# sebrahimi1988/dss-ml-at-scale

Measured on NVIDIA H100. Metric: series fitted+forecast/sec, higher is better.
Workload: dtype f32

## Files before the change

dss-ml-at-scale_b200/csrc/fit_tc.cu:

```cuda
#include "mmf_internal.cuh"
#include "sm90_ptx.cuh"

namespace mmf {
namespace {

using namespace sm90;

constexpr int TILE_M = 128;
constexpr int KC = 32;
constexpr int NGROUPS = 2;
constexpr int FOLD_CHUNKS = 18;
constexpr int MAX_PRED = 64;
constexpr int BULK_MAX_PRED = 28;
constexpr int Y_STAGE_BYTES = TILE_M * KC * 4;
constexpr int AT_STAGE_BYTES = 2 * P * KC * 4;
constexpr int THREADS = 416;
constexpr int WARP_EPI0 = 8, WARP_PROD = 12;

template <int STAGES, int OBUF, bool SE = false>
struct SmemLayoutT {
  static constexpr int y = 0;
  static constexpr int at = y + STAGES * Y_STAGE_BYTES;
  static constexpr int apred = at + STAGES * AT_STAGE_BYTES;
  static constexpr int ostage = apred + MAX_PRED * P * 4;
  static constexpr int acc = ostage + OBUF * TILE_M * BULK_MAX_PRED * 4;
  static constexpr int nm = acc + 2 * NGROUPS * TILE_M * P * 4;
  static constexpr int cc = nm + 2 * NGROUPS * TILE_M * 2;
  static constexpr int bars = cc + NGROUPS * 2 * TILE_M * 4;
  static constexpr int n_bars = 2 * STAGES + 4;
  static constexpr int ss = bars + n_bars * 8;
  static constexpr int sfac = ss + (SE ? 2 * NGROUPS * TILE_M * 8 : 0);
  static constexpr int total = sfac + (SE ? MAX_PRED * 4 : 0);
  static_assert(total + 1024 <= 232448, "exceeds the 227 KB of shared memory a CTA can opt into");
};

__device__ __forceinline__ float dot16(const float* __restrict__ arow, const float (&g)[P], float s) {
  const float4* ap = reinterpret_cast<const float4*>(arow);
  const float4 a0 = ap[0], a1 = ap[1], a2 = ap[2], a3 = ap[3];
  s = fmaf(a0.x, g[0], s);  s = fmaf(a0.y, g[1], s);  s = fmaf(a0.z, g[2], s);  s = fmaf(a0.w, g[3], s);
  s = fmaf(a1.x, g[4], s);  s = fmaf(a1.y, g[5], s);  s = fmaf(a1.z, g[6], s);  s = fmaf(a1.w, g[7], s);
  s = fmaf(a2.x, g[8], s);  s = fmaf(a2.y, g[9], s);  s = fmaf(a2.z, g[10], s); s = fmaf(a2.w, g[11], s);
  s = fmaf(a3.x, g[12], s); s = fmaf(a3.y, g[13], s); s = fmaf(a3.z, g[14], s); s = fmaf(a3.w, g[15], s);
  return s;
}

__device__ __forceinline__ float centring_constant(const float* __restrict__ yrow, int t_fit) {
  float v[8];
  if (t_fit >= 8) {
    const float4 a = __ldg(reinterpret_cast<const float4*>(yrow)), b = __ldg(reinterpret_cast<const float4*>(yrow) + 1);
    v[0] = a.x; v[1] = a.y; v[2] = a.z; v[3] = a.w; v[4] = b.x; v[5] = b.y; v[6] = b.z; v[7] = b.w;
  } else {
#pragma unroll
    for (int i = 0; i < 8; ++i) v[i] = i < t_fit ? __ldg(yrow + i) : __int_as_float(0x7fc00000);
  }
  float c = v[7];
#pragma unroll
  for (int i = 6; i >= 0; --i) c = ((__float_as_uint(v[i]) & 0x7f800000u) != 0x7f800000u) ? v[i] : c;
  return c;
}

__device__ __forceinline__ bool is_finite_bits(float x) { return (__float_as_uint(x) & 0x7f800000u) != 0x7f800000u; }

__device__ __forceinline__ void bt_write_moments(const BtArgs& bt, int k, int grp, int64_t n, const TileRec& tr, int frow0,
                                                 int t4, const float (&acc)[2][P], bool folded, const float* sacc) {
#pragma unroll
  for (int h = 0; h < 2; ++h)
#pragma unroll
    for (int j = 0; j < 2; ++j) {
      const int rt = 64 * h + frow0 + 8 * j;
      if (rt >= tr.nrows) continue;
      float* __restrict__ dst = bt.mom + (((int64_t)k * 2 + grp) * n + tr.row0 + rt) * P + 2 * t4;
#pragma unroll
      for (int i = 0; i < 2; ++i) {
        const int q = 4 * i + 2 * j;
        float2 v = make_float2(acc[h][q] + acc[h][q + P / 2], acc[h][q + 1] + acc[h][q + 1 + P / 2]);
        if (folded) {
          const float2 o = *reinterpret_cast<const float2*>(sacc + rt * P + 8 * i + 2 * t4);
          v.x = o.x + v.x; v.y = o.y + v.y;
        }
        *reinterpret_cast<float2*>(dst + 8 * i) = v;
      }
    }
}

__device__ __forceinline__ float lds32(uint32_t addr) {
  float v;
  asm volatile("ld.shared.f32 %0, [%1];" : "=f"(v) : "r"(addr));
  return v;
}

template <int STAGES, int OBUF, bool MULTI, bool SE = false, bool BT = false>
__global__ void __launch_bounds__(THREADS, 1)
fit_tc_kernel(const __grid_constant__ TcLaunch tl, const DesignView d, const FitArgs a,
              uint32_t* __restrict__ pending_count, const int n_tiles, const int n_chunks, const MultiView mv,
              const SeArgs se, const BtArgs bt) {
  static_assert(!SE || !MULTI, "standard errors are built for the single-calendar launch");
  static_assert(!BT || !(MULTI || SE), "backtests are built for the single-calendar launch");
  using SmemLayout = SmemLayoutT<STAGES, OBUF, SE>;
  auto tile_rec = [&](int ti) -> TileRec {
    if (MULTI) {
      if (ti >= n_tiles) return TileRec{0, 0, 0, 1};
      const int4 v = __ldg(reinterpret_cast<const int4*>(mv.tiles) + ti);
      return TileRec{v.x, v.y, v.z, v.w};
    }
    const int64_t left = a.n - (int64_t)ti * TILE_M;
    return TileRec{ti * TILE_M, (int)(left >= TILE_M ? TILE_M : (left > 0 ? left : 0)), 0, n_chunks};
  };
  auto tfit_of = [&](const TileRec& t) -> int { return MULTI ? __ldg(&mv.cals[t.cal].t_fit) : d.t_fit; };
  extern __shared__ unsigned char smem_dyn[];
  unsigned char* smem = reinterpret_cast<unsigned char*>((reinterpret_cast<uintptr_t>(smem_dyn) + 1023) & ~uintptr_t(1023));
  const uint32_t sbase = smem_u32(smem);
  const uint32_t s_y = sbase + SmemLayout::y;
  const uint32_t s_at = sbase + SmemLayout::at;
  float* s_apred = reinterpret_cast<float*>(smem + SmemLayout::apred);
  float* s_ostage = reinterpret_cast<float*>(smem + SmemLayout::ostage);
  float* s_acc = reinterpret_cast<float*>(smem + SmemLayout::acc);
  uint16_t* s_nm = reinterpret_cast<uint16_t*>(smem + SmemLayout::nm);
  float* s_cc = reinterpret_cast<float*>(smem + SmemLayout::cc);
  double* s_ss = reinterpret_cast<double*>(smem + SmemLayout::ss);
  float* s_sfac = reinterpret_cast<float*>(smem + SmemLayout::sfac);
#ifdef MMF_TC_NO_COLLECT
  const bool collect = false;
#else
  const bool collect = a.recs != nullptr && d.t_fit <= 65535;
#endif
  const uint32_t s_bars = sbase + SmemLayout::bars;
  auto bar_full = [&](int s) { return s_bars + 8u * s; };
  auto bar_empty = [&](int s) { return s_bars + 8u * (STAGES + s); };
  auto bar_accfull = [&](int b) { return s_bars + 8u * (2 * STAGES + b); };
  auto bar_accempty = [&](int b) { return s_bars + 8u * (2 * STAGES + 2 + b); };

  const int warp = threadIdx.x >> 5;
  const int lane = threadIdx.x & 31;

  if (blockIdx.x == 0 && threadIdx.x == 0 && a.zero_next != nullptr) {
#pragma unroll
    for (int i = 0; i < CTR_WORDS; ++i) a.zero_next[i] = 0u;
  }
  if (warp == WARP_PROD) {
    if (lane == 0) {
      for (int s = 0; s < STAGES; ++s) {
        mbar_init(bar_full(s), 1);
        mbar_init(bar_empty(s), 4);
      }
      for (int b = 0; b < 2; ++b) {
        mbar_init(bar_accfull(b), NGROUPS * 128);
        mbar_init(bar_accempty(b), 4);
      }
      fence_mbar_init();
      prefetch_tensormap(tl.tmap_y);
      prefetch_tensormap(tl.tmap_at);
    }
  } else if (warp >= WARP_EPI0) {
    if (!a.skip_pred && !MULTI)
      for (int i = threadIdx.x - WARP_EPI0 * 32; i < a.n_pred * P; i += 128)
        s_apred[i] = __ldg(d.apred + (size_t)a.pred_start * P + i);
    if (SE && !a.skip_pred)
      for (int i = threadIdx.x - WARP_EPI0 * 32; i < a.n_pred; i += 128) s_sfac[i] = __ldg(se.sfac + a.pred_start + i);
  }
  __syncthreads();
  if (threadIdx.x == 0) pdl_launch_dependents();

  if (warp == WARP_PROD) {
    int stage = 0;
    uint32_t phase = 0;
    int last_cal = -1;
    for (int tile = blockIdx.x; tile < n_tiles; tile += gridDim.x) {
      const TileRec tr = tile_rec(tile);
      const void* tmy = MULTI ? static_cast<const void*>(mv.tmaps_y + (size_t)tr.cal * 128) : static_cast<const void*>(tl.tmap_y);
      if (MULTI && tr.cal != last_cal) { fence_tensormap_acquire(tmy); last_cal = tr.cal; }
      const int at_row = MULTI ? tr.cal * 2 * P : 0;
      for (int ch = 0; ch < tr.n_chunks; ++ch) {
        mbar_wait(bar_empty(stage), phase ^ 1u);
        tma_load_2d_x2_elect(bar_full(stage), Y_STAGE_BYTES + AT_STAGE_BYTES,
                             s_y + stage * Y_STAGE_BYTES, tmy, ch * KC, tr.row0, L2_EVICT_FIRST,
                             s_at + stage * AT_STAGE_BYTES, tl.tmap_at, ch * KC, at_row,
                             MULTI ? L2_EVICT_NORMAL : L2_EVICT_LAST);
        if (++stage == STAGES) { stage = 0; phase ^= 1u; }
      }
    }
  } else if (warp < NGROUPS * 4) {
    const int grp = warp >> 2;
    const int r = threadIdx.x & 127;
    const uint32_t row_off = static_cast<uint32_t>(r) * 128u;
    const uint32_t sw = static_cast<uint32_t>(r & 7);
    const int g8 = lane >> 2, t4 = lane & 3;
    const int frow0 = 16 * (warp & 3) + g8;
    float* __restrict__ s_c = s_cc + grp * 2 * TILE_M;
    uint32_t gc = 0;
    int tile = blockIdx.x;
    TileRec tr = tile_rec(tile);
    TileRec trn = tile_rec(tile + (int)gridDim.x);
    auto load_c = [&](int tl_, const TileRec& t) -> float {
      return (d.has_constant && tl_ < n_tiles && r < t.nrows)
                 ? centring_constant(a.y + (int64_t)(t.row0 + r) * a.ld_y, tfit_of(t)) : 0.f;
    };
    float c = load_c(tile, tr);
    float c_next = load_c(tile + (int)gridDim.x, trn);
    for (int lt = 0; tile < n_tiles; ++lt) {
      const bool bad = collect && !is_finite_bits(c);
      if (bad) c = 0.f;
      s_c[(lt & 1) * TILE_M + r] = c;
      named_bar_sync(4 + grp, 128);
      float cf[2][2];
#pragma unroll
      for (int h = 0; h < 2; ++h)
#pragma unroll
        for (int j = 0; j < 2; ++j) cf[h][j] = s_c[(lt & 1) * TILE_M + 64 * h + frow0 + 8 * j];
      float acc[2][P];
#pragma unroll
      for (int h = 0; h < 2; ++h)
#pragma unroll
        for (int i = 0; i < P; ++i) acc[h][i] = 0.f;
      const bool scan = collect && (!MULTI || r < tr.nrows);
      const int seg = (grp ^ (int)gc) & 1;
      int nm = 0;
      unsigned long long packq = 0ull;
      const int ab = lt & 1;
      float* __restrict__ sacc = s_acc + (ab * NGROUPS + grp) * TILE_M * P;
      auto sacc_at = [&](int h, int j, int i) {
        return reinterpret_cast<float2*>(sacc + (64 * h + frow0 + 8 * j) * P + 8 * i + 2 * t4);
      };
      bool folded = false;
      int since_fold = 0;
      double ssq[2][2] = {{0.0, 0.0}, {0.0, 0.0}};
      for (int ch = seg; ch < tr.n_chunks; ch += NGROUPS) {
        const uint32_t k = gc + static_cast<uint32_t>(ch);
        const int stage = static_cast<int>(k % STAGES);
        mbar_wait(bar_full(stage), (k / STAGES) & 1u);
        const uint32_t sy = s_y + stage * Y_STAGE_BYTES;
        if (scan) {
          const uint32_t rowp = sy + row_off;
          float4 v[8];
#pragma unroll
          for (int q = 0; q < 8; ++q) v[q] = lds128(rowp + ((static_cast<uint32_t>(q) ^ sw) << 4));
          float chk = 0.f;
#pragma unroll
          for (int q = 0; q < 8; ++q) {
            chk = fmaf(v[q].x, 0.f, chk); chk = fmaf(v[q].y, 0.f, chk);
            chk = fmaf(v[q].z, 0.f, chk); chk = fmaf(v[q].w, 0.f, chk);
          }
          if (!(chk == 0.f)) {
            unsigned gaps = 0u;
#pragma unroll
            for (int q = 0; q < 8; ++q)
              gaps |= (is_finite_bits(v[q].x) ? 0u : 1u << (4 * q)) | (is_finite_bits(v[q].y) ? 0u : 2u << (4 * q)) |
                      (is_finite_bits(v[q].z) ? 0u : 4u << (4 * q)) | (is_finite_bits(v[q].w) ? 0u : 8u << (4 * q));
            uint16_t* __restrict__ mt = a.recs[(int64_t)tr.row0 + r].miss_t + seg * SOLVE_SEG;
            const int tbase = ch * KC;
            while (gaps) {
              const int pos = __ffs(gaps) - 1;
              gaps &= gaps - 1u;
              packq = (packq >> 16) | (static_cast<unsigned long long>(tbase + pos) << 48);
              ++nm;
              if ((nm & 3) == 0 && nm <= SOLVE_SEG) *reinterpret_cast<unsigned long long*>(mt + nm - 4) = packq;
              if constexpr (BT) if (nm == SOLVE_SEG + 1)
                reinterpret_cast<uint16_t*>(&a.recs[(int64_t)tr.row0 + r].ss)[seg] = static_cast<uint16_t>(tbase + pos);
            }
          }
        }
        uint32_t ahi[2][KC / 8][4], alo[2][KC / 8][4];
        const int lim = d.t_fit - ch * KC;
#pragma unroll
        for (int h = 0; h < 2; ++h)
#pragma unroll
          for (int j = 0; j < 2; ++j) {
            const uint32_t rowp = sy + static_cast<uint32_t>(64 * h + frow0 + 8 * j) * 128u + t4 * 4;
            float part = 0.f;
#pragma unroll
            for (int kk = 0; kk < KC / 8; ++kk)
#pragma unroll
              for (int hf = 0; hf < 2; ++hf) {
                float x = lds32(rowp + ((static_cast<uint32_t>(2 * kk + hf) ^ static_cast<uint32_t>(g8)) << 4));
                if (collect) x = is_finite_bits(x) ? x : cf[h][j];
                const float rr = x - cf[h][j];
                const uint32_t hb = __float_as_uint(rr) & 0xFFFFE000u;
                ahi[h][kk][j + 2 * hf] = hb;
                alo[h][kk][j + 2 * hf] = __float_as_uint(rr - __uint_as_float(hb));
                if (SE) {
                  const float rs = 4 * (2 * kk + hf) + t4 < lim ? rr : 0.f;
                  part = fmaf(rs, rs, part);
                }
              }
// ... 99 lines not shown
                if (folded) { const float2 o = *sacc_at(h, j, i); f.x = o.x + f.x; f.y = o.y + f.y; }
                *sacc_at(h, j, i) = f;
              }
#pragma unroll
          for (int h = 0; h < 2; ++h)
#pragma unroll
            for (int i = 0; i < P; ++i) acc[h][i] = 0.f;
          folded = true;
          since_fold = 0;
        }
      }
      if (scan && (nm & 3) != 0 && nm < SOLVE_SEG) {
        uint16_t* __restrict__ mt = a.recs[(int64_t)tr.row0 + r].miss_t + seg * SOLVE_SEG;
        *reinterpret_cast<unsigned long long*>(mt + (nm & ~3)) = packq >> (16 * (4 - (nm & 3)));
      }
      if constexpr (BT) {
        const int s_end = ((tr.n_chunks - 1 - seg) / NGROUPS * NGROUPS + seg + 1) * KC;
        uint32_t rest = 0;
#pragma unroll
        for (int k = 0; k < MMF_BT_MAX_ORIGINS - 1; ++k) rest |= (bt.t_orig[k] != INT32_MAX && bt.t_orig[k] >= s_end ? 1u : 0u) << k;
        while (rest) {
          const int k = __ffs(rest) - 1;
          rest &= rest - 1u;
          bt_write_moments(bt, k, grp, a.n, tr, frow0, t4, acc, folded, sacc);
        }
      }
      if (!folded) mbar_wait(bar_accempty(ab), ((lt >> 1) & 1) ^ 1u);
#pragma unroll
      for (int h = 0; h < 2; ++h)
#pragma unroll
        for (int j = 0; j < 2; ++j)
#pragma unroll
          for (int i = 0; i < 2; ++i) {
            const int q = 4 * i + 2 * j;
            float2 v = make_float2(acc[h][q] + acc[h][q + P / 2], acc[h][q + 1] + acc[h][q + 1 + P / 2]);
            if (folded) { const float2 o = *sacc_at(h, j, i); v.x = o.x + v.x; v.y = o.y + v.y; }
            *sacc_at(h, j, i) = v;
          }
      if (SE) {
#pragma unroll
        for (int h = 0; h < 2; ++h)
#pragma unroll
          for (int j = 0; j < 2; ++j) {
            double v = ssq[h][j];
            v += __shfl_xor_sync(0xffffffffu, v, 1);
            v += __shfl_xor_sync(0xffffffffu, v, 2);
            if (t4 == 0) s_ss[(ab * NGROUPS + grp) * TILE_M + 64 * h + frow0 + 8 * j] = v;
          }
      }
      const int cnt = nm > 0x7ffe ? 0x7ffe : nm;
      s_nm[(ab * NGROUPS + seg) * TILE_M + r] = static_cast<uint16_t>(cnt | (bad ? 0x8000 : 0));
      mbar_arrive(bar_accfull(ab));
      gc += static_cast<uint32_t>(tr.n_chunks);
      tile += gridDim.x;
      tr = trn;
      trn = tile_rec(tile + (int)gridDim.x);
      c = c_next;
      c_next = load_c(tile + (int)gridDim.x, trn);
    }
  } else {
    const int r = threadIdx.x & 127;
    bool vec_out = (a.n_pred % 4 == 0) && (a.ld_out % 4 == 0) && ((reinterpret_cast<uintptr_t>(a.out) & 15u) == 0);
    for (int i = 0; i + 1 < a.n_out; ++i) vec_out = vec_out && ((reinterpret_cast<uintptr_t>(a.out_more[i]) & 15u) == 0);
#ifdef MMF_TC_NO_BULK
    const bool bulk = false;
#else
    const bool bulk = !a.skip_pred && vec_out && a.out_multimem != 1 && a.ld_out == a.n_pred && a.n_pred <= BULK_MAX_PRED;
#endif
    const uint32_t s_ostage_u32 = smem_u32(s_ostage);
    const bool se_vec = SE && (a.n_pred % 4 == 0) && (se.ld_se % 4 == 0) &&
                        ((reinterpret_cast<uintptr_t>(se.out_se) & 15u) == 0);
    int lt = 0;
    int cur_cal = MULTI ? -1 : 0;
    uint32_t kept_mask = d.kept_mask;
    int t_fit_c = d.t_fit;
    for (int tile = blockIdx.x; tile < n_tiles; tile += gridDim.x, ++lt) {
      const int ab = lt & 1;
      const TileRec tr = tile_rec(tile);
      const int64_t row = (int64_t)tr.row0 + r;
      const bool live = r < tr.nrows;
      if (MULTI && tr.cal != cur_cal) {
        const int4* cp = reinterpret_cast<const int4*>(mv.cals + tr.cal);
        const int4 m0 = __ldg(cp), m1 = __ldg(cp + 1);
        t_fit_c = m0.x;
        kept_mask = static_cast<uint32_t>(m0.w);
        if (!a.skip_pred) {
          named_bar_sync(2, 128);
          const float* __restrict__ src = d.apred + (size_t)(m1.x + m1.y) * P;
          for (int i = threadIdx.x - WARP_EPI0 * 32; i < a.n_pred * P; i += 128) s_apred[i] = __ldg(src + i);
          named_bar_sync(2, 128);
        }
        cur_cal = tr.cal;
      }
      float c = (d.has_constant && live) ? centring_constant(a.y + row * a.ld_y, t_fit_c) : 0.f;
      mbar_wait(bar_accfull(ab), (lt >> 1) & 1);
      float g[P];
      {
        const float4* p0 = reinterpret_cast<const float4*>(s_acc + (ab * NGROUPS + 0) * TILE_M * P + r * P);
        const float4* p1 = reinterpret_cast<const float4*>(s_acc + (ab * NGROUPS + 1) * TILE_M * P + r * P);
#pragma unroll
        for (int q = 0; q < P / 4; ++q) {
          const float4 u = p0[q], w = p1[q];
          g[4 * q] = u.x + w.x; g[4 * q + 1] = u.y + w.y; g[4 * q + 2] = u.z + w.z; g[4 * q + 3] = u.w + w.w;
        }
      }
      const unsigned f0 = s_nm[(ab * NGROUPS + 0) * TILE_M + r], f1 = s_nm[(ab * NGROUPS + 1) * TILE_M + r];
      const double ss = SE ? s_ss[(ab * NGROUPS + 0) * TILE_M + r] + s_ss[(ab * NGROUPS + 1) * TILE_M + r] : 0.0;
      if constexpr (BT) {
        __syncwarp();
        if (lane == 0) mbar_arrive(bar_accempty(ab));
        for (int k = 0; k < bt.n_origin; ++k) {
          const bool last = k == bt.n_origin - 1;
          const int4 m0 = __ldg(reinterpret_cast<const int4*>(bt.cals + k));
          const int tk = m0.x;
          float gk[P];
          if (last || !live) {
#pragma unroll
            for (int p = 0; p < P; ++p) gk[p] = g[p];
          } else {
            const float4* p0 = reinterpret_cast<const float4*>(bt.mom + (((int64_t)k * NGROUPS + 0) * a.n + row) * P);
            const float4* p1 = reinterpret_cast<const float4*>(bt.mom + (((int64_t)k * NGROUPS + 1) * a.n + row) * P);
#pragma unroll
            for (int q = 0; q < P / 4; ++q) {
              const float4 u = p0[q], w = p1[q];
              gk[4 * q] = u.x + w.x; gk[4 * q + 1] = u.y + w.y; gk[4 * q + 2] = u.z + w.z; gk[4 * q + 3] = u.w + w.w;
            }
          }
          const SolveRec* __restrict__ src = collect ? a.recs + row : nullptr;
          int n0 = f0 & 0x7fff, n1 = f1 & 0x7fff;
          bool over = false;
          if (collect && !last && live && (n0 | n1) != 0) {
#pragma unroll
            for (int sg = 0; sg < 2; ++sg) {
              const int tot = sg ? n1 : n0;
              const uint16_t* mt = src->miss_t + sg * SOLVE_SEG;
              const int have = tot < SOLVE_SEG ? tot : SOLVE_SEG;
              int cnt = 0;
              while (cnt < have && mt[cnt] < tk) ++cnt;
              if (cnt == SOLVE_SEG && tot > SOLVE_SEG && reinterpret_cast<const uint16_t*>(&src->ss)[sg] < tk) over = true;
              if (sg) n1 = cnt; else n0 = cnt;
            }
          }
          bool general = false;
          if (collect)
            general = ((f0 | f1) & 0x8000u) != 0u || over || n0 > SOLVE_SEG || n1 > SOLVE_SEG || 2 * (n0 + n1) > tk;
          bool finite = true;
#pragma unroll
          for (int p = 0; p < P; ++p) {
// ... 65 lines not shown
      if (lane == 0) mbar_arrive(bar_accempty(ab));
      int nm0 = 0, nm1 = 0;
      bool general = false;
      if (collect) {
        nm0 = f0 & 0x7fff; nm1 = f1 & 0x7fff;
        general = ((f0 | f1) & 0x8000u) != 0u || nm0 > SOLVE_SEG || nm1 > SOLVE_SEG || 2 * (nm0 + nm1) > t_fit_c;
        if (general) c = 0.f;
      }
      bool finite = true;
#pragma unroll
      for (int p = 0; p < P; ++p) {
        finite = finite && is_finite_bits(g[p]);
        if (!((kept_mask >> p) & 1u)) g[p] = 0.f;
      }
      const bool pend = live && (!finite || general);
      const bool defer = live && !pend && (nm0 + nm1) > 0;
      const unsigned pm = __ballot_sync(0xffffffffu, pend);
      if (lane == 0 && pm != 0u) {
        atomicAdd(pending_count, __popc(pm));
        if (MULTI) atomicAdd(mv.pending_by_cal + tr.cal, __popc(pm));
      }
      const unsigned dm = __ballot_sync(0xffffffffu, defer);
      if (dm != 0u) {
        unsigned base = 0;
        if (lane == 0) base = atomicAdd(a.rec_count, __popc(dm));
        base = __shfl_sync(0xffffffffu, base, 0);
        if (defer) {
          SolveRec& rec = a.recs[row];
          float4* bp = reinterpret_cast<float4*>(rec.b);
          bp[0] = make_float4(g[0], g[1], g[2], g[3]);    bp[1] = make_float4(g[4], g[5], g[6], g[7]);
          bp[2] = make_float4(g[8], g[9], g[10], g[11]);  bp[3] = make_float4(g[12], g[13], g[14], g[15]);
          rec.c = c;
          if (SE) rec.ss = static_cast<float>(ss);
          rec.nm[0] = static_cast<uint16_t>(nm0);
          rec.nm[1] = static_cast<uint16_t>(nm1);
          rec.cal = tr.cal;
          const unsigned slot = base + __popc(dm & ((1u << lane) - 1u));
          if (slot < a.rec_cap) a.rec_rows[slot] = row;
        }
      }
      if (bulk) {
        const int ob = OBUF > 1 ? (lt % OBUF) : 0;
        if (warp == WARP_EPI0) { if (OBUF > 1) bulk_wait_read1_elect(); else bulk_wait_read_elect(); }
        named_bar_sync(1, 128);
        float* __restrict__ srow = s_ostage + ob * (TILE_M * BULK_MAX_PRED) + r * a.n_pred;
        for (int k = 0; k < a.n_pred; k += 4) {
          float o[4];
#pragma unroll
          for (int w = 0; w < 4; ++w) o[w] = dot16(s_apred + (k + w) * P, g, c);
          *reinterpret_cast<float4*>(srow + k) = make_float4(o[0], o[1], o[2], o[3]);
        }
        fence_proxy_async_smem();
        named_bar_sync(1, 128);
        if (warp == WARP_EPI0) {
          const uint32_t bytes = static_cast<uint32_t>(tr.nrows) * a.n_pred * 4u;
          const int64_t off = (int64_t)tr.row0 * a.n_pred;
          const uint32_t src = s_ostage_u32 + static_cast<uint32_t>(ob) * (TILE_M * BULK_MAX_PRED * 4);
          bulk_store_hint_elect(reinterpret_cast<uint64_t>(a.out + off), src, bytes, L2_EVICT_FIRST);
          const int n_peer = a.n_out - 1;
          int j = n_peer > 1 ? tile % n_peer : 0;
          for (int i = 0; i < n_peer; ++i) {
            bulk_store_elect(reinterpret_cast<uint64_t>(a.out_more[j] + off), src, bytes);
            if (++j == n_peer) j = 0;
          }
          bulk_commit_elect();
        }
      } else if (live && !pend && !defer && !a.skip_pred) {
        const int64_t off = row * a.ld_out;
        if (vec_out) {
          for (int k = 0; k < a.n_pred; k += 4) {
            float o[4];
#pragma unroll
            for (int w = 0; w < 4; ++w) o[w] = dot16(s_apred + (k + w) * P, g, c);
            store_out4(a, off + k, make_float4(o[0], o[1], o[2], o[3]));
          }
        } else {
          for (int k = 0; k < a.n_pred; ++k) store_out1(a, off + k, dot16(s_apred + k * P, g, c));
        }
      }
      if (live) {
        if (!pend && !defer) {
          if (a.out_gamma != nullptr) {
            float4* gp = reinterpret_cast<float4*>(a.out_gamma + row * P);
            gp[0] = make_float4(g[0], g[1], g[2], g[3]);    gp[1] = make_float4(g[4], g[5], g[6], g[7]);
            gp[2] = make_float4(g[8], g[9], g[10], g[11]);  gp[3] = make_float4(g[12], g[13], g[14], g[15]);
            a.out_c[row] = c;
          }
          if (a.out_beta != nullptr) {
            float* __restrict__ br = a.out_beta + row * P;
            for (int p = 0; p < P; ++p) {
              float s = (p == 0 && d.has_constant) ? c : 0.f;
#pragma unroll
              for (int q = 0; q < P; ++q) s = fmaf(__ldg(d.w + p * P + q), g[q], s);
              br[p] = s;
            }
          }
          if (SE) {
            double bg = 0.0;
#pragma unroll
            for (int p = 0; p < P; ++p) bg = fma(static_cast<double>(g[p]), static_cast<double>(g[p]), bg);
            const int dof = t_fit_c - __popc(kept_mask);
            const double rss = fmax(ss - bg, 0.0);
            const float sig = dof > 0 ? static_cast<float>(sqrt(rss / dof)) : __int_as_float(0x7fc00000);
            se.sigma[row] = sig;
            if (se.dof != nullptr) se.dof[row] = dof;
            if (se.out_se != nullptr && !a.skip_pred) {
              float* __restrict__ srow = se.out_se + row * se.ld_se;
              int k = 0;
              if (se_vec)
                for (; k < a.n_pred; k += 4)
                  __stcs(reinterpret_cast<float4*>(srow + k),
                         make_float4(sig * s_sfac[k], sig * s_sfac[k + 1], sig * s_sfac[k + 2], sig * s_sfac[k + 3]));
              for (; k < a.n_pred; ++k) __stcs(srow + k, sig * s_sfac[k]);
            }
          }
          a.status[row] = MMF_STATUS_OK;
        } else {
          a.status[row] = pend ? MMF_STATUS_PENDING : MMF_STATUS_DEFERRED;
        }
      }
    }
    if (bulk && warp == WARP_EPI0) bulk_wait_all_elect();
  }
}

}

bool fit_tc_supported(const DesignView& d, const FitArgs& a, const char** why) {
  const char* w = nullptr;
  if (!a.skip_pred && a.n_pred > MAX_PRED) w = "n_pred > 64 needs the fit + predict_tc_kernel pair";
  else if (a.n_pred < 1) w = "n_pred < 1";
  else if (a.ld_y % 4 != 0) w = "ld_y not a multiple of 4 floats (TMA needs 16-B row pitch)";
  else if ((reinterpret_cast<uintptr_t>(a.y) & 15u) != 0) w = "y not 16-B aligned";
  else if (d.t_fit < 1) w = "t_fit < 1";
  else if (a.n > (int64_t)0x7fffffff - TILE_M) w = "n too large for 32-bit TMA coordinates";
  if (why) *why = w;
  return w == nullptr;
}

template <int STAGES, int OBUF, bool MULTI, bool SE = false, bool BT = false>
static cudaError_t launch_variant(const DesignView& d, const FitArgs& a, const TcLaunch& tl, uint32_t* pending_count,
                                  int sm_count, cudaStream_t s, int n_tiles, int n_chunks, const MultiView& mv,
                                  const SeArgs& se = SeArgs{}, const BtArgs& bt = BtArgs{}) {
  const size_t smem = SmemLayoutT<STAGES, OBUF, SE>::total + 1024;
  cudaError_t e = cudaFuncSetAttribute(fit_tc_kernel<STAGES, OBUF, MULTI, SE, BT>, cudaFuncAttributeMaxDynamicSharedMemorySize, (int)smem);
  if (e != cudaSuccess) return e;
  const int grid = n_tiles < sm_count ? n_tiles : sm_count;
  fit_tc_kernel<STAGES, OBUF, MULTI, SE, BT><<<grid, THREADS, smem, s>>>(tl, d, a, pending_count, n_tiles, n_chunks, mv, se, bt);
  return cudaGetLastError();
}

cudaError_t launch_fit_tc(const DesignView& d, const FitArgs& a, const TcLaunch& tl, uint32_t* pending_count,
                          int sm_count, cudaStream_t s, int variant, const MultiView* multi) {
  if (a.n <= 0) return cudaSuccess;
  if (multi != nullptr)
    return launch_variant<8, 1, true>(d, a, tl, pending_count, sm_count, s, multi->n_tiles, 2, *multi);
  const int n_tiles = (int)((a.n + TILE_M - 1) / TILE_M);
  const int n_chunks = d.t_pad / KC;
  const MultiView none{};
  return variant == 2 ? launch_variant<6, 2, false>(d, a, tl, pending_count, sm_count, s, n_tiles, n_chunks, none)
                      : launch_variant<8, 1, false>(d, a, tl, pending_count, sm_count, s, n_tiles, n_chunks, none);
}

cudaError_t launch_fit_tc_se(const DesignView& d, const FitArgs& a, const TcLaunch& tl, uint32_t* pending_count,
                             int sm_count, cudaStream_t s, const SeArgs& se) {
  if (a.n <= 0) return cudaSuccess;
  const int n_tiles = (int)((a.n + TILE_M - 1) / TILE_M);
  return launch_variant<8, 1, false, true>(d, a, tl, pending_count, sm_count, s, n_tiles, d.t_pad / KC, MultiView{}, se);
}

cudaError_t launch_fit_tc_bt(const DesignView& d, const FitArgs& a, const TcLaunch& tl, uint32_t* pending_count,
                             int sm_count, cudaStream_t s, const BtArgs& bt) {
// ... 8 lines not shown
```

dss-ml-at-scale_b200/csrc/mmf_internal.cuh:

```cuda
#pragma once
#include <cuda_runtime.h>
#include <stdint.h>
#include "../../include/mmf.h"

namespace mmf {

constexpr int P = MMF_P;
constexpr int NPAIR = P * (P + 1) / 2;

struct DesignView {
  const float4* a4;
  const float*  at;
  const float*  apred;
  const float*  w;
  int32_t n_rows;
  int32_t n_rows_pad;
  int32_t t_fit;
  int32_t t_pad;
  uint32_t kept_mask;
  int32_t has_constant;
};

struct CalMeta {
  int32_t t_fit;
// ... 45 lines not shown
  int32_t n_pred;
  float* out;
  int64_t ld_out;
  float* out_more[MAX_OUT - 1];
  int32_t n_out;
  int32_t out_multimem;
  float* out_gamma;
  float* out_c;
  int32_t skip_pred;
  float* out_beta;
  int32_t* status;
  SolveRec* recs;
  int64_t* rec_rows;
  uint32_t* rec_count;
  uint32_t rec_cap;
  int32_t only_pending;
  const uint32_t* pending_count;
  uint32_t* zero_next;
  int64_t row_base;
  int32_t cal_id;
};

struct SeArgs {
  float* out_se;
  int64_t ld_se;
  float* sigma;
  int32_t* dof;
  const float* sfac;
};

struct BtArgs {
  const CalMeta* cals;
  const float* pred;
  const float* tmat;
  float* mom;
  SolveRec* recs;
  int64_t* rec_rows;
  uint32_t* rec_count;
  uint32_t* pending;
  int64_t out_kstride;
  int64_t st_kstride;
  int32_t n_origin;
  int32_t t_orig[MMF_BT_MAX_ORIGINS - 1];
};

cudaError_t launch_fit_warp(const DesignView& d, const FitArgs& a, int sm_count, cudaStream_t s,
                            const SeArgs* se = nullptr);
size_t fit_warp_smem_bytes(const DesignView& d, int* smem_rows);

cudaError_t launch_solve_rows(const DesignView& d, const FitArgs& a, int sm_count, cudaStream_t s,
                              const CalMeta* cals = nullptr, const SeArgs* se = nullptr);
cudaError_t launch_se_outer(const FitArgs& a, const SeArgs& se, int sm_count, cudaStream_t s);
constexpr int CTR_WORDS = 8;

struct PredictLaunch {
  alignas(64) unsigned char tmap_bhi[128];
  alignas(64) unsigned char tmap_blo[128];
  alignas(64) unsigned char tmap_out[128];
  int32_t n_tma;
};
struct PredUnit {
  int32_t row0, nrows;
  int32_t cal;
  int32_t ch;
  int32_t b_row;
  int32_t row_in_map;
  int32_t pad_[2];
};
static_assert(sizeof(PredUnit) == 32, "PredUnit is two 16-B loads");
cudaError_t launch_predict_tc(const DesignView& d, const FitArgs& a, const PredictLaunch& pl, int sm_count,
                              cudaStream_t s, const PredUnit* units = nullptr, int64_t n_units_multi = 0,
                              const unsigned char* tmaps_out = nullptr);

struct TcLaunch {
  alignas(64) unsigned char tmap_y[128];
  alignas(64) unsigned char tmap_at[128];
};
cudaError_t launch_fit_tc(const DesignView& d, const FitArgs& a, const TcLaunch& tl,
                          uint32_t* pending_count, int sm_count, cudaStream_t s, int variant = 0,
                          const MultiView* multi = nullptr);
cudaError_t launch_fit_tc_se(const DesignView& d, const FitArgs& a, const TcLaunch& tl, uint32_t* pending_count,
                             int sm_count, cudaStream_t s, const SeArgs& se);
cudaError_t launch_fit_tc_bt(const DesignView& d, const FitArgs& a, const TcLaunch& tl, uint32_t* pending_count,
                             int sm_count, cudaStream_t s, const BtArgs& bt);
bool fit_tc_supported(const DesignView& d, const FitArgs& a, const char** why);

struct ScoreArgs {
  const float* pred;
  int64_t ld_pred, pred_kstride;
  const float* y;
  int64_t ld_y;
  const CalMeta* cals;
  float* metrics;
  int32_t* count;
  int64_t out_kstride;
  int64_t n;
  int32_t n_origin, horizon;
};
cudaError_t launch_bt_score(const ScoreArgs& sa, int sm_count, cudaStream_t s);

constexpr int MMF_MAX_CAND = 8;
struct SelectArgs {
  int32_t n_hold;
  int32_t n_cand;
  int32_t cand[MMF_MAX_CAND];
  int32_t* out_choice;
// ... 55 lines not shown
```

dss-ml-at-scale_b200/csrc/sm90_ptx.cuh:

```cuda
#pragma once
#include <cuda_runtime.h>
#include <stdint.h>

namespace sm90 {

__device__ __forceinline__ uint32_t smem_u32(const void* p) {
  return static_cast<uint32_t>(__cvta_generic_to_shared(p));
}

__device__ __forceinline__ void mbar_init(uint32_t bar, uint32_t count) {
  asm volatile("mbarrier.init.shared::cta.b64 [%0], %1;" ::"r"(bar), "r"(count) : "memory");
}
__device__ __forceinline__ void fence_mbar_init() {
  asm volatile("fence.mbarrier_init.release.cluster;" ::: "memory");
}
__device__ __forceinline__ void fence_proxy_async_smem() {
  asm volatile("fence.proxy.async.shared::cta;" ::: "memory");
}
__device__ __forceinline__ void mbar_arrive(uint32_t bar) {
  asm volatile("mbarrier.arrive.shared::cta.b64 _, [%0];" ::"r"(bar) : "memory");
}
__device__ __forceinline__ void mbar_expect_tx(uint32_t bar, uint32_t bytes) {
  asm volatile("mbarrier.arrive.expect_tx.shared::cta.b64 _, [%0], %1;" ::"r"(bar), "r"(bytes) : "memory");
}
// ... 78 lines not shown
      : "memory");
}
__device__ __forceinline__ void tma_load_2d_elect(uint32_t bar, uint32_t tx_bytes, uint32_t dst, const void* tmap,
                                                  int32_t c0, int32_t c1, uint64_t hint) {
  asm volatile(
      "{\n\t.reg .pred pe;\n\t"
      "elect.sync _|pe, 0xffffffff;\n\t"
      "@pe mbarrier.arrive.expect_tx.shared::cta.b64 _, [%0], %1;\n\t"
      "@pe cp.async.bulk.tensor.2d.shared::cluster.global.mbarrier::complete_tx::bytes.L2::cache_hint"
      " [%2], [%3, {%4, %5}], [%0], %6;\n\t}"
      ::"r"(bar), "r"(tx_bytes), "r"(dst), "l"(reinterpret_cast<uint64_t>(tmap)), "r"(c0), "r"(c1), "l"(hint)
      : "memory");
}

__device__ __forceinline__ void bulk_store_elect(uint64_t dst_global, uint32_t src_smem, uint32_t bytes) {
  asm volatile(
      "{\n\t.reg .pred pe;\n\t"
      "elect.sync _|pe, 0xffffffff;\n\t"
      "@pe cp.async.bulk.global.shared::cta.bulk_group [%0], [%1], %2;\n\t}"
      ::"l"(dst_global), "r"(src_smem), "r"(bytes)
      : "memory");
}
__device__ __forceinline__ void bulk_store_hint_elect(uint64_t dst_global, uint32_t src_smem, uint32_t bytes, uint64_t hint) {
  asm volatile(
      "{\n\t.reg .pred pe;\n\t"
      "elect.sync _|pe, 0xffffffff;\n\t"
      "@pe cp.async.bulk.global.shared::cta.bulk_group.L2::cache_hint [%0], [%1], %2, %3;\n\t}"
      ::"l"(dst_global), "r"(src_smem), "r"(bytes), "l"(hint)
      : "memory");
}
__device__ __forceinline__ void bulk_commit_elect() {
  asm volatile(
      "{\n\t.reg .pred pe;\n\t"
      "elect.sync _|pe, 0xffffffff;\n\t"
      "@pe cp.async.bulk.commit_group;\n\t}" ::: "memory");
}
__device__ __forceinline__ void bulk_wait_read_elect() {
  asm volatile(
      "{\n\t.reg .pred pe;\n\t"
      "elect.sync _|pe, 0xffffffff;\n\t"
      "@pe cp.async.bulk.wait_group.read 0;\n\t}" ::: "memory");
}
__device__ __forceinline__ void bulk_wait_read1_elect() {
  asm volatile(
      "{\n\t.reg .pred pe;\n\t"
      "elect.sync _|pe, 0xffffffff;\n\t"
      "@pe cp.async.bulk.wait_group.read 1;\n\t}" ::: "memory");
}
__device__ __forceinline__ void bulk_wait_all_elect() {
  asm volatile(
      "{\n\t.reg .pred pe;\n\t"
      "elect.sync _|pe, 0xffffffff;\n\t"
      "@pe cp.async.bulk.wait_group 0;\n\t}" ::: "memory");
}
__device__ __forceinline__ void named_bar_sync(uint32_t id, uint32_t nthreads) {
  asm volatile("bar.sync %0, %1;" ::"r"(id), "r"(nthreads) : "memory");
}

__device__ __forceinline__ void tma_store_2d_elect(const void* tmap, uint32_t src_smem, int32_t c0, int32_t c1) {
  asm volatile(
      "{\n\t.reg .pred pe;\n\t"
      "elect.sync _|pe, 0xffffffff;\n\t"
      "@pe cp.async.bulk.tensor.2d.global.shared::cta.bulk_group [%0, {%2, %3}], [%1];\n\t}"
      ::"l"(reinterpret_cast<uint64_t>(tmap)), "r"(src_smem), "r"(c0), "r"(c1)
      : "memory");
}

__device__ __forceinline__ uint64_t gmma_desc_k(uint32_t smem_addr, uint32_t sbo_bytes, uint32_t layout) {
  uint64_t d = 0;
  d |= static_cast<uint64_t>((smem_addr & 0x3FFFFu) >> 4);
  d |= static_cast<uint64_t>(1) << 16;
  d |= static_cast<uint64_t>(sbo_bytes >> 4) << 32;
  d |= static_cast<uint64_t>(layout) << 62;
  return d;
}
__device__ __forceinline__ uint64_t gmma_desc_k_sw128(uint32_t smem_addr) { return gmma_desc_k(smem_addr, 1024, 1); }
__device__ __forceinline__ uint64_t gmma_desc_k_sw64(uint32_t smem_addr) { return gmma_desc_k(smem_addr, 512, 2); }

__device__ __forceinline__ void wgmma_fence() { asm volatile("wgmma.fence.sync.aligned;" ::: "memory"); }
__device__ __forceinline__ void wgmma_commit() { asm volatile("wgmma.commit_group.sync.aligned;" ::: "memory"); }
template <int N>
__device__ __forceinline__ void wgmma_wait() { asm volatile("wgmma.wait_group.sync.aligned %0;" ::"n"(N) : "memory"); }
template <int N>
__device__ __forceinline__ void wgmma_fence_regs(float (&d)[N]) {
#pragma unroll
  for (int i = 0; i < N; ++i) asm volatile("" : "+f"(d[i])::"memory");
}

__device__ __forceinline__ void wgmma_m64n32k8_tf32_rs(float (&d)[16], const uint32_t (&a)[4], uint64_t b_desc) {
  asm volatile(
      "wgmma.mma_async.sync.aligned.m64n32k8.f32.tf32.tf32 "
      "{%0, %1, %2, %3, %4, %5, %6, %7, %8, %9, %10, %11, %12, %13, %14, %15}, {%16, %17, %18, %19}, %20, 1, 1, 1;"
      : "+f"(d[0]), "+f"(d[1]), "+f"(d[2]), "+f"(d[3]), "+f"(d[4]), "+f"(d[5]), "+f"(d[6]), "+f"(d[7]), "+f"(d[8]), "+f"(d[9]), "+f"(d[10]), "+f"(d[11]), "+f"(d[12]), "+f"(d[13]), "+f"(d[14]), "+f"(d[15])
      : "r"(a[0]), "r"(a[1]), "r"(a[2]), "r"(a[3]), "l"(b_desc));
}
__device__ __forceinline__ void wgmma_m64n128k8_tf32_rs(float (&d)[64], const uint32_t (&a)[4], uint64_t b_desc) {
  asm volatile(
      "wgmma.mma_async.sync.aligned.m64n128k8.f32.tf32.tf32 "
      "{%0, %1, %2, %3, %4, %5, %6, %7, %8, %9, %10, %11, %12, %13, %14, %15, %16, %17, %18, %19, %20, %21, %22, %23, %24, %25, %26, %27, %28, %29, %30, %31, %32, %33, %34, %35, %36, %37, %38, %39, %40, %41, %42, %43, %44, %45, %46, %47, %48, %49, %50, %51, %52, %53, %54, %55, %56, %57, %58, %59, %60, %61, %62, %63}, {%64, %65, %66, %67}, %68, 1, 1, 1;"
      : "+f"(d[0]), "+f"(d[1]), "+f"(d[2]), "+f"(d[3]), "+f"(d[4]), "+f"(d[5]), "+f"(d[6]), "+f"(d[7]), "+f"(d[8]), "+f"(d[9]), "+f"(d[10]), "+f"(d[11]), "+f"(d[12]), "+f"(d[13]), "+f"(d[14]), "+f"(d[15]), "+f"(d[16]), "+f"(d[17]), "+f"(d[18]), "+f"(d[19]), "+f"(d[20]), "+f"(d[21]), "+f"(d[22]), "+f"(d[23]), "+f"(d[24]), "+f"(d[25]), "+f"(d[26]), "+f"(d[27]), "+f"(d[28]), "+f"(d[29]), "+f"(d[30]), "+f"(d[31]), "+f"(d[32]), "+f"(d[33]), "+f"(d[34]), "+f"(d[35]), "+f"(d[36]), "+f"(d[37]), "+f"(d[38]), "+f"(d[39]), "+f"(d[40]), "+f"(d[41]), "+f"(d[42]), "+f"(d[43]), "+f"(d[44]), "+f"(d[45]), "+f"(d[46]), "+f"(d[47]), "+f"(d[48]), "+f"(d[49]), "+f"(d[50]), "+f"(d[51]), "+f"(d[52]), "+f"(d[53]), "+f"(d[54]), "+f"(d[55]), "+f"(d[56]), "+f"(d[57]), "+f"(d[58]), "+f"(d[59]), "+f"(d[60]), "+f"(d[61]), "+f"(d[62]), "+f"(d[63])
      : "r"(a[0]), "r"(a[1]), "r"(a[2]), "r"(a[3]), "l"(b_desc));
}

__device__ __forceinline__ void sts128(uint32_t addr, float4 v) {
  asm volatile("st.shared.v4.f32 [%0], {%1, %2, %3, %4};" ::"r"(addr), "f"(v.x), "f"(v.y), "f"(v.z), "f"(v.w) : "memory");
}
// ... 8 lines not shown
```

Baseline: 577.7 million.

## Add dynamic tile claiming ring, compute centring constants from smem, store outputs directly

Replaces the static grid-stride tile loop with a producer-driven dynamic scheduler: the TMA warp claims tiles through a global atomic counter and broadcasts them to the compute and epilogue warps via an mbarrier-guarded shared ring. The centring constant now comes from the first Y chunk already resident in shared memory instead of separate global loads in both the math and epilogue warps, and it is shared through a new barrier. Output stores switch from a single-thread bulk async copy to all 128 epilogue threads doing vectorized stores with an evict-first L2 policy, and the Y TMA load hint changes to evict-normal. These changes aim to balance load and cut redundant global reads, but they add atomics, extra barrier waits and a change in which status path writes. The MULTI path also now uses KC instead of the per-calendar t_fit.

```diff
diff --git a/dss-ml-at-scale_b200/csrc/fit_tc.cu b/dss-ml-at-scale_b200/csrc/fit_tc.cu
--- a/dss-ml-at-scale_b200/csrc/fit_tc.cu
+++ b/dss-ml-at-scale_b200/csrc/fit_tc.cu
@@ -15,6 +15,7 @@
 constexpr int Y_STAGE_BYTES = TILE_M * KC * 4;
 constexpr int AT_STAGE_BYTES = 2 * P * KC * 4;
 constexpr int THREADS = 416;
+constexpr int TILE_RING = 4;
 constexpr int WARP_EPI0 = 8, WARP_PROD = 12;
 
 template <int STAGES, int OBUF, bool SE = false>
@@ -26,8 +27,9 @@
   static constexpr int acc = ostage + OBUF * TILE_M * BULK_MAX_PRED * 4;
   static constexpr int nm = acc + 2 * NGROUPS * TILE_M * P * 4;
   static constexpr int cc = nm + 2 * NGROUPS * TILE_M * 2;
-  static constexpr int bars = cc + NGROUPS * 2 * TILE_M * 4;
-  static constexpr int n_bars = 2 * STAGES + 4;
+  static constexpr int tiles = cc + 2 * TILE_M * 4;
+  static constexpr int bars = tiles + TILE_RING * 4;
+  static constexpr int n_bars = 2 * STAGES + 6 + 2 * TILE_RING;
   static constexpr int ss = bars + n_bars * 8;
   static constexpr int sfac = ss + (SE ? 2 * NGROUPS * TILE_M * 8 : 0);
   static constexpr int total = sfac + (SE ? MAX_PRED * 4 : 0);
@@ -44,22 +46,15 @@
   return s;
 }
 
-__device__ __forceinline__ float centring_constant(const float* __restrict__ yrow, int t_fit) {
-  float v[8];
-  if (t_fit >= 8) {
-    const float4 a = __ldg(reinterpret_cast<const float4*>(yrow)), b = __ldg(reinterpret_cast<const float4*>(yrow) + 1);
-    v[0] = a.x; v[1] = a.y; v[2] = a.z; v[3] = a.w; v[4] = b.x; v[5] = b.y; v[6] = b.z; v[7] = b.w;
-  } else {
-#pragma unroll
-    for (int i = 0; i < 8; ++i) v[i] = i < t_fit ? __ldg(yrow + i) : __int_as_float(0x7fc00000);
-  }
-  float c = v[7];
-#pragma unroll
-  for (int i = 6; i >= 0; --i) c = ((__float_as_uint(v[i]) & 0x7f800000u) != 0x7f800000u) ? v[i] : c;
+__device__ __forceinline__ bool is_finite_bits(float x) { return (__float_as_uint(x) & 0x7f800000u) != 0x7f800000u; }
+
+__device__ __forceinline__ float centring_constant(const float4& a, const float4& b, int t_fit) {
+  const float v[8] = {a.x, a.y, a.z, a.w, b.x, b.y, b.z, b.w};
+  float c = t_fit > 7 ? v[7] : __int_as_float(0x7fc00000);
+#pragma unroll
+  for (int i = 6; i >= 0; --i) c = (i < t_fit && is_finite_bits(v[i])) ? v[i] : c;
   return c;
 }
-
-__device__ __forceinline__ bool is_finite_bits(float x) { return (__float_as_uint(x) & 0x7f800000u) != 0x7f800000u; }
 
 __device__ __forceinline__ void bt_write_moments(const BtArgs& bt, int k, int grp, int64_t n, const TileRec& tr, int frow0,
                                                  int t4, const float (&acc)[2][P], bool folded, const float* sacc) {
@@ -106,7 +101,6 @@
     const int64_t left = a.n - (int64_t)ti * TILE_M;
     return TileRec{ti * TILE_M, (int)(left >= TILE_M ? TILE_M : (left > 0 ? left : 0)), 0, n_chunks};
   };
-  auto tfit_of = [&](const TileRec& t) -> int { return MULTI ? __ldg(&mv.cals[t.cal].t_fit) : d.t_fit; };
   extern __shared__ unsigned char smem_dyn[];
   unsigned char* smem = reinterpret_cast<unsigned char*>((reinterpret_cast<uintptr_t>(smem_dyn) + 1023) & ~uintptr_t(1023));
   const uint32_t sbase = smem_u32(smem);
@@ -125,13 +119,24 @@
   const bool collect = a.recs != nullptr && d.t_fit <= 65535;
 #endif
   const uint32_t s_bars = sbase + SmemLayout::bars;
+  const int warp = threadIdx.x >> 5;
+  const int lane = threadIdx.x & 31;
   auto bar_full = [&](int s) { return s_bars + 8u * s; };
   auto bar_empty = [&](int s) { return s_bars + 8u * (STAGES + s); };
   auto bar_accfull = [&](int b) { return s_bars + 8u * (2 * STAGES + b); };
   auto bar_accempty = [&](int b) { return s_bars + 8u * (2 * STAGES + 2 + b); };
-
-  const int warp = threadIdx.x >> 5;
-  const int lane = threadIdx.x & 31;
+  auto bar_cc = [&](int b) { return s_bars + 8u * (2 * STAGES + 4 + b); };
+  auto bar_tfull = [&](int s) { return s_bars + 8u * (2 * STAGES + 6 + s); };
+  auto bar_tempty = [&](int s) { return s_bars + 8u * (2 * STAGES + 6 + TILE_RING + s); };
+  int* s_tiles = reinterpret_cast<int*>(smem + SmemLayout::tiles);
+  auto take_tile = [&](int lt) -> int {
+    const int sl = lt % TILE_RING;
+    mbar_wait(bar_tfull(sl), (lt / TILE_RING) & 1);
+    const int t = *reinterpret_cast<volatile int*>(s_tiles + sl);
+    __syncwarp();
+    if (lane == 0) mbar_arrive(bar_tempty(sl));
+    return t;
+  };
 
   if (blockIdx.x == 0 && threadIdx.x == 0 && a.zero_next != nullptr) {
 #pragma unroll
@@ -146,6 +151,11 @@
       for (int b = 0; b < 2; ++b) {
         mbar_init(bar_accfull(b), NGROUPS * 128);
         mbar_init(bar_accempty(b), 4);
+        mbar_init(bar_cc(b), 128);
+      }
+      for (int sl = 0; sl < TILE_RING; ++sl) {
+        mbar_init(bar_tfull(sl), 1);
+        mbar_init(bar_tempty(sl), NGROUPS * 4 + 4);
       }
       fence_mbar_init();
       prefetch_tensormap(tl.tmap_y);
@@ -165,7 +175,20 @@
     int stage = 0;
     uint32_t phase = 0;
     int last_cal = -1;
-    for (int tile = blockIdx.x; tile < n_tiles; tile += gridDim.x) {
+    uint32_t* claim_ctr = pending_count + CTR_TILE_CLAIM;
+    int tile = blockIdx.x;
+    for (int lt = 0;; ++lt) {
+      const int sl = lt % TILE_RING;
+      mbar_wait(bar_tempty(sl), ((lt / TILE_RING) & 1) ^ 1u);
+      const bool more = tile < n_tiles;
+      uint32_t claim = 0;
+      if (lane == 0) {
+        if (more) claim = atomicAdd(claim_ctr, 1u);
+        s_tiles[sl] = more ? tile : -1;
+        mbar_arrive(bar_tfull(sl));
+      }
+      __syncwarp();
+      if (!more) break;
       const TileRec tr = tile_rec(tile);
       const void* tmy = MULTI ? static_cast<const void*>(mv.tmaps_y + (size_t)tr.cal * 128) : static_cast<const void*>(tl.tmap_y);
       if (MULTI && tr.cal != last_cal) { fence_tensormap_acquire(tmy); last_cal = tr.cal; }
@@ -173,11 +196,12 @@
       for (int ch = 0; ch < tr.n_chunks; ++ch) {
         mbar_wait(bar_empty(stage), phase ^ 1u);
         tma_load_2d_x2_elect(bar_full(stage), Y_STAGE_BYTES + AT_STAGE_BYTES,
-                             s_y + stage * Y_STAGE_BYTES, tmy, ch * KC, tr.row0, L2_EVICT_FIRST,
+                             s_y + stage * Y_STAGE_BYTES, tmy, ch * KC, tr.row0, L2_EVICT_NORMAL,
                              s_at + stage * AT_STAGE_BYTES, tl.tmap_at, ch * KC, at_row,
                              MULTI ? L2_EVICT_NORMAL : L2_EVICT_LAST);
         if (++stage == STAGES) { stage = 0; phase ^= 1u; }
       }
+      tile = static_cast<int>(gridDim.x + __shfl_sync(0xffffffffu, claim, 0));
     }
   } else if (warp < NGROUPS * 4) {
     const int grp = warp >> 2;
@@ -186,27 +210,13 @@
     const uint32_t sw = static_cast<uint32_t>(r & 7);
     const int g8 = lane >> 2, t4 = lane & 3;
     const int frow0 = 16 * (warp & 3) + g8;
-    float* __restrict__ s_c = s_cc + grp * 2 * TILE_M;
     uint32_t gc = 0;
-    int tile = blockIdx.x;
-    TileRec tr = tile_rec(tile);
-    TileRec trn = tile_rec(tile + (int)gridDim.x);
-    auto load_c = [&](int tl_, const TileRec& t) -> float {
-      return (d.has_constant && tl_ < n_tiles && r < t.nrows)
-                 ? centring_constant(a.y + (int64_t)(t.row0 + r) * a.ld_y, tfit_of(t)) : 0.f;
-    };
-    float c = load_c(tile, tr);
-    float c_next = load_c(tile + (int)gridDim.x, trn);
-    for (int lt = 0; tile < n_tiles; ++lt) {
-      const bool bad = collect && !is_finite_bits(c);
-      if (bad) c = 0.f;
-      s_c[(lt & 1) * TILE_M + r] = c;
-      named_bar_sync(4 + grp, 128);
+    for (int lt = 0;; ++lt) {
+      const int tile = take_tile(lt);
+      if (tile < 0) break;
+      const TileRec tr = tile_rec(tile);
+      bool bad = false;
       float cf[2][2];
-#pragma unroll
-      for (int h = 0; h < 2; ++h)
-#pragma unroll
-        for (int j = 0; j < 2; ++j) cf[h][j] = s_c[(lt & 1) * TILE_M + 64 * h + frow0 + 8 * j];
       float acc[2][P];
 #pragma unroll
       for (int h = 0; h < 2; ++h)
@@ -229,6 +239,24 @@
         const int stage = static_cast<int>(k % STAGES);
         mbar_wait(bar_full(stage), (k / STAGES) & 1u);
         const uint32_t sy = s_y + stage * Y_STAGE_BYTES;
+        if (ch == seg) {
+          if (seg == 0) {
+            mbar_wait(bar_accempty(ab), ((lt >> 1) & 1) ^ 1u);
+            float c = 0.f;
+            if (d.has_constant && r < tr.nrows) {
+              const uint32_t rowp = sy + row_off;
+              c = centring_constant(lds128(rowp + (sw << 4)), lds128(rowp + ((1u ^ sw) << 4)), MULTI ? KC : d.t_fit);
+            }
+            bad = collect && !is_finite_bits(c);
+            s_cc[ab * TILE_M + r] = bad ? 0.f : c;
+            mbar_arrive(bar_cc(ab));
+          }
+          mbar_wait(bar_cc(ab), (lt >> 1) & 1);
+#pragma unroll
+          for (int h = 0; h < 2; ++h)
+#pragma unroll
+            for (int j = 0; j < 2; ++j) cf[h][j] = s_cc[ab * TILE_M + 64 * h + frow0 + 8 * j];
+        }
         if (scan) {
           const uint32_t rowp = sy + row_off;
           float4 v[8];
@@ -434,11 +462,6 @@
       s_nm[(ab * NGROUPS + seg) * TILE_M + r] = static_cast<uint16_t>(cnt | (bad ? 0x8000 : 0));
       mbar_arrive(bar_accfull(ab));
       gc += static_cast<uint32_t>(tr.n_chunks);
-      tile += gridDim.x;
-      tr = trn;
-      trn = tile_rec(tile + (int)gridDim.x);
-      c = c_next;
-      c_next = load_c(tile + (int)gridDim.x, trn);
     }
   } else {
     const int r = threadIdx.x & 127;
@@ -450,13 +473,16 @@
     const bool bulk = !a.skip_pred && vec_out && a.out_multimem != 1 && a.ld_out == a.n_pred && a.n_pred <= BULK_MAX_PRED;
 #endif
     const uint32_t s_ostage_u32 = smem_u32(s_ostage);
+    const uint64_t l2_policy = l2_evict_first_policy();
     const bool se_vec = SE && (a.n_pred % 4 == 0) && (se.ld_se % 4 == 0) &&
                         ((reinterpret_cast<uintptr_t>(se.out_se) & 15u) == 0);
     int lt = 0;
     int cur_cal = MULTI ? -1 : 0;
     uint32_t kept_mask = d.kept_mask;
     int t_fit_c = d.t_fit;
-    for (int tile = blockIdx.x; tile < n_tiles; tile += gridDim.x, ++lt) {
+    for (;; ++lt) {
+      const int tile = take_tile(lt);
+      if (tile < 0) break;
       const int ab = lt & 1;
       const TileRec tr = tile_rec(tile);
       const int64_t row = (int64_t)tr.row0 + r;
@@ -474,8 +500,8 @@
         }
         cur_cal = tr.cal;
       }
-      float c = (d.has_constant && live) ? centring_constant(a.y + row * a.ld_y, t_fit_c) : 0.f;
       mbar_wait(bar_accfull(ab), (lt >> 1) & 1);
+      float c = s_cc[ab * TILE_M + r];
       float g[P];
       {
         const float4* p0 = reinterpret_cast<const float4*>(s_acc + (ab * NGROUPS + 0) * TILE_M * P + r * P);
@@ -647,11 +673,12 @@
         }
         fence_proxy_async_smem();
         named_bar_sync(1, 128);
+        const uint32_t bytes = static_cast<uint32_t>(tr.nrows) * a.n_pred * 4u;
+        const int64_t off = (int64_t)tr.row0 * a.n_pred;
+        const uint32_t src = s_ostage_u32 + static_cast<uint32_t>(ob) * (TILE_M * BULK_MAX_PRED * 4);
+        for (uint32_t i = r; i < bytes / 16u; i += 128u)
+          stg128_hint(reinterpret_cast<float4*>(a.out + off) + i, lds128(src + 16u * i), l2_policy);
         if (warp == WARP_EPI0) {
-          const uint32_t bytes = static_cast<uint32_t>(tr.nrows) * a.n_pred * 4u;
-          const int64_t off = (int64_t)tr.row0 * a.n_pred;
-          const uint32_t src = s_ostage_u32 + static_cast<uint32_t>(ob) * (TILE_M * BULK_MAX_PRED * 4);
-          bulk_store_hint_elect(reinterpret_cast<uint64_t>(a.out + off), src, bytes, L2_EVICT_FIRST);
           const int n_peer = a.n_out - 1;
           int j = n_peer > 1 ? tile % n_peer : 0;
           for (int i = 0; i < n_peer; ++i) {
@@ -709,10 +736,8 @@
               for (; k < a.n_pred; ++k) __stcs(srow + k, sig * s_sfac[k]);
             }
           }
-          a.status[row] = MMF_STATUS_OK;
-        } else {
-          a.status[row] = pend ? MMF_STATUS_PENDING : MMF_STATUS_DEFERRED;
-        }
+        }
+        stg32_hint(a.status + row, pend ? MMF_STATUS_PENDING : (defer ? MMF_STATUS_DEFERRED : MMF_STATUS_OK), l2_policy);
       }
     }
     if (bulk && warp == WARP_EPI0) bulk_wait_all_elect();
diff --git a/dss-ml-at-scale_b200/csrc/mmf_internal.cuh b/dss-ml-at-scale_b200/csrc/mmf_internal.cuh
--- a/dss-ml-at-scale_b200/csrc/mmf_internal.cuh
+++ b/dss-ml-at-scale_b200/csrc/mmf_internal.cuh
@@ -121,6 +121,7 @@
                               const CalMeta* cals = nullptr, const SeArgs* se = nullptr);
 cudaError_t launch_se_outer(const FitArgs& a, const SeArgs& se, int sm_count, cudaStream_t s);
 constexpr int CTR_WORDS = 8;
+constexpr int CTR_TILE_CLAIM = 2;
 
 struct PredictLaunch {
   alignas(64) unsigned char tmap_bhi[128];
diff --git a/dss-ml-at-scale_b200/csrc/sm90_ptx.cuh b/dss-ml-at-scale_b200/csrc/sm90_ptx.cuh
--- a/dss-ml-at-scale_b200/csrc/sm90_ptx.cuh
+++ b/dss-ml-at-scale_b200/csrc/sm90_ptx.cuh
@@ -154,6 +154,18 @@
       "{\n\t.reg .pred pe;\n\t"
       "elect.sync _|pe, 0xffffffff;\n\t"
       "@pe cp.async.bulk.wait_group 0;\n\t}" ::: "memory");
+}
+__device__ __forceinline__ uint64_t l2_evict_first_policy() {
+  uint64_t p;
+  asm volatile("createpolicy.fractional.L2::evict_first.b64 %0, 1.0;" : "=l"(p));
+  return p;
+}
+__device__ __forceinline__ void stg128_hint(void* dst, float4 v, uint64_t policy) {
+  asm volatile("st.global.L2::cache_hint.v4.f32 [%0], {%1, %2, %3, %4}, %5;"
+               ::"l"(dst), "f"(v.x), "f"(v.y), "f"(v.z), "f"(v.w), "l"(policy) : "memory");
+}
+__device__ __forceinline__ void stg32_hint(void* dst, uint32_t v, uint64_t policy) {
+  asm volatile("st.global.L2::cache_hint.b32 [%0], %1, %2;" ::"l"(dst), "r"(v), "l"(policy) : "memory");
 }
 __device__ __forceinline__ void named_bar_sync(uint32_t id, uint32_t nthreads) {
   asm volatile("bar.sync %0, %1;" ::"r"(id), "r"(nthreads) : "memory");
```

Measured after the change: 616.7 million, median of 6. 6.7% higher.
